# SamsungLabs/fcaf3d

Hardware: AMD Instinct MI355X
Metric: scenes/sec fwd+bwd, ScanNet 100k-pt 2cm voxels, 1/2/4/8 MI355X (higher is better)
Workload: dtype f32

## Files before the change

### fcaf3d_amd/csrc/conv.hip

```cpp
#include "fc_common.h"
#include "../../include/fcaf3d_hip.h"
#ifdef FC_TRACE
__device__ unsigned long long* g_trace_buf_lds;
__device__ int g_trace_cap_lds;
extern "C" int fc_debug_trace_lds(unsigned long long* buf, int cap) {
  FC_HIP(hipMemcpyToSymbol(HIP_SYMBOL(g_trace_buf_lds), &buf, sizeof(buf)));
  FC_HIP(hipMemcpyToSymbol(HIP_SYMBOL(g_trace_cap_lds), &cap, sizeof(cap)));
  return FC_OK;
}
#define TR_BUF g_trace_buf_lds
#define TR_CAP g_trace_cap_lds
#endif
#include "fc_trace.h"

typedef float f32x16 __attribute__((ext_vector_type(16)));
typedef float f32x2 __attribute__((ext_vector_type(2)));
typedef float f32x4 __attribute__((ext_vector_type(4)));

__device__ __attribute__((aligned(16))) float g_zero_row[64];

__device__ int g_fc_prio;
extern "C" int fc_debug_set_prio(int mode) {
  FC_HIP(hipMemcpyToSymbol(HIP_SYMBOL(g_fc_prio), &mode, sizeof(mode)));
  return FC_OK;
// ... 149 lines not shown
  *reinterpret_cast<f32x4*>(out + o * Cout + c4 * 4) = a;
}

__host__ __device__ static inline int fc_stat_rb(int64_t n) { return n <= 1024 ? 16 : (n <= 4096 ? 64 : 32); }

__device__ __forceinline__ void stat_block_reduce(f32x4 a1, f32x4 a2, float* __restrict__ stats, int C, f32x4* sm ) {
  const int lane = threadIdx.x & 15, rl = threadIdx.x >> 4;
  sm[(rl * 2 + 0) * 16 + lane] = a1;
  sm[(rl * 2 + 1) * 16 + lane] = a2;
  __syncthreads();
  if (rl < 2) {
    f32x4 t = {0.f, 0.f, 0.f, 0.f};
#pragma unroll
    for (int q = 0; q < 16; ++q) t += sm[(q * 2 + rl) * 16 + lane];
    *reinterpret_cast<f32x4*>(stats + ((int64_t)blockIdx.x * 2 + rl) * C + blockIdx.y * 64 + lane * 4) = t;
  }
}

struct StatCh { f32x4 mu, is, ga, be; bool bwd, from_y, has_add; int act; };
__device__ __forceinline__ StatCh stat_channels(const X6Epi& epi, int c) {
  StatCh p;
  p.bwd = epi.bn_x != nullptr;
  p.act = epi.act;
  p.from_y = p.bwd && epi.bn_y != nullptr && epi.act != 0;
  p.has_add = p.bwd && epi.add != nullptr;
  p.mu = f32x4{0.f, 0.f, 0.f, 0.f}; p.is = f32x4{1.f, 1.f, 1.f, 1.f}; p.ga = p.is; p.be = p.mu;
  if (p.bwd) {
    p.mu = *reinterpret_cast<const f32x4*>(epi.mean + c);
    const f32x4 va = *reinterpret_cast<const f32x4*>(epi.var + c);
#pragma unroll
    for (int j = 0; j < 4; ++j) p.is[j] = 1.f / sqrtf(va[j] + epi.eps);
    if (epi.gamma) p.ga = *reinterpret_cast<const f32x4*>(epi.gamma + c);
    if (epi.beta) p.be = *reinterpret_cast<const f32x4*>(epi.beta + c);
  }
  return p;
}
__device__ __forceinline__ void stat_accumulate(const StatCh& p, const X6Epi& epi, const f32x4& a, int64_t at, f32x4& a1, f32x4& a2) {
  f32x4 xv = {0.f, 0.f, 0.f, 0.f}, av = xv, yv = xv;
  if (p.bwd) xv = *reinterpret_cast<const f32x4*>(epi.bn_x + at);
  if (p.has_add) av = *reinterpret_cast<const f32x4*>(epi.add + at);
  if (p.from_y) yv = *reinterpret_cast<const f32x4*>(epi.bn_y + at);
#pragma unroll
  for (int j = 0; j < 4; ++j) {
    float t1, t2;
    x6_epi_terms(p.bwd, p.bwd ? av[j] + a[j] : a[j], xv[j], p.mu[j], p.is[j], p.ga[j], p.be[j], p.act, p.from_y, yv[j], t1, t2);
    a1[j] += t1;
    a2[j] += t2;
  }
}

__global__ __launch_bounds__(256) void k_sum_parts_stats(const float* __restrict__ part, float* __restrict__ out, int64_t n, int C, int S,
                                                         int RB, X6Epi epi) {
  __shared__ f32x4 sm[16 * 2 * 16];
  const int lane = threadIdx.x & 15, rl = threadIdx.x >> 4;
  const int64_t r0 = (int64_t)blockIdx.x * RB;
  const int c = blockIdx.y * 64 + lane * 4;
  const StatCh p = stat_channels(epi, c);
  f32x4 a1 = {0.f, 0.f, 0.f, 0.f}, a2 = a1;
  for (int64_t r = r0 + rl; r < r0 + RB && r < n; r += 16) {
    f32x4 a = *reinterpret_cast<const f32x4*>(part + r * C + c);
    for (int z = 1; z < S; ++z) a += *reinterpret_cast<const f32x4*>(part + ((int64_t)z * n + r) * C + c);
    *reinterpret_cast<f32x4*>(out + r * C + c) = a;
    stat_accumulate(p, epi, a, r * C + c, a1, a2);
  }
  stat_block_reduce(a1, a2, epi.stats, C, sm);
}

__global__ __launch_bounds__(256) void k_sum_pairs_stats(const float* __restrict__ part, const int* __restrict__ pos, float* __restrict__ out,
                                                         int64_t n_out, int K, int Cout, int RB, X6Epi epi) {
  __shared__ f32x4 sm[16 * 2 * 16];
  const int lane = threadIdx.x & 15, rl = threadIdx.x >> 4;
  const int64_t r0 = (int64_t)blockIdx.x * RB;
  const int c = blockIdx.y * 64 + lane * 4;
  const StatCh p = stat_channels(epi, c);
  f32x4 a1 = {0.f, 0.f, 0.f, 0.f}, a2 = a1;
  const int64_t rend = (r0 + RB < n_out) ? r0 + RB : n_out;
  for (int64_t o = r0 + rl; o < rend; o += 32) {
    const int64_t o2 = o + 16;
    const bool two = o2 < rend;
    f32x4 a = {0.f, 0.f, 0.f, 0.f}, b = a;
    for (int k0 = 0; k0 < K; k0 += 9) {
      int j[9], j2[9];
#pragma unroll
      for (int u = 0; u < 9; ++u) {
        j[u] = k0 + u < K ? pos[(int64_t)(k0 + u) * n_out + o] : -1;
        j2[u] = (two && k0 + u < K) ? pos[(int64_t)(k0 + u) * n_out + o2] : -1;
      }
      f32x4 v[9], v2[9];
#pragma unroll
      for (int u = 0; u < 9; ++u) {
        const float* src = j[u] >= 0 ? part + ((int64_t)(k0 + u) * n_out + j[u]) * Cout + c : g_zero_row + lane * 4;
        const float* src2 = j2[u] >= 0 ? part + ((int64_t)(k0 + u) * n_out + j2[u]) * Cout + c : g_zero_row + lane * 4;
        v[u] = *reinterpret_cast<const f32x4*>(src);
        v2[u] = *reinterpret_cast<const f32x4*>(src2);
      }
#pragma unroll
      for (int u = 0; u < 9; ++u) {
        if (j[u] >= 0) a += v[u];
        if (j2[u] >= 0) b += v2[u];
      }
    }
    *reinterpret_cast<f32x4*>(out + o * Cout + c) = a;
    stat_accumulate(p, epi, a, o * Cout + c, a1, a2);
    if (two) {
      *reinterpret_cast<f32x4*>(out + o2 * Cout + c) = b;
      stat_accumulate(p, epi, b, o2 * Cout + c, a1, a2);
    }
  }
  stat_block_reduce(a1, a2, epi.stats, Cout, sm);
}

static_assert(STEM_CIN == 3 && STEM_COUT == 64 && BK == 32, "conv_route.h spells these shapes out");

struct ConvArgs {
  const float *in, *W; const int *nbr, *out_index, *cnt; float* dst;
  int64_t n_rows; int K, Cin, Cout; X6Epi epi; hipStream_t stream;
};
#define FC_LAUNCH(...) __VA_ARGS__<<<grid, 256, 0, a.stream>>>(a.in, a.W, a.nbr, a.out_index, a.cnt, a.dst, a.n_rows, a.K, a.Cin, a.Cout)
#define FC_LAUNCH_EPI(...) __VA_ARGS__<<<grid, 256, 0, a.stream>>>(a.in, a.W, a.nbr, a.out_index, a.cnt, a.dst, a.n_rows, a.K, a.Cin, a.Cout, a.epi)

template <int BM, int BN, int WM>
static void launch_conv_fp32(const ConvRoute& r, const ConvArgs& a, dim3 grid) {
#define FC_LAUNCH_MFMA(KERNEL)                                                                                              \
  do { if (r.wsrc == FC_WSRC_FP32_T) FC_LAUNCH(KERNEL<BM, BN, 32, true, WM, true>); else if (a.nbr) FC_LAUNCH(KERNEL<BM, BN, 32, true, WM>); \
       else FC_LAUNCH(KERNEL<BM, BN, 32, false, WM>); } while (0)
  if (r.family == FC_FAM_MFMA) FC_LAUNCH_MFMA(k_conv_mfma);
  if constexpr (BM >= 128) {
    if (r.family == FC_FAM_MFMA_P) FC_LAUNCH_MFMA(k_conv_mfma_p);
    if (r.family == FC_FAM_GLDS) { if (a.nbr) FC_LAUNCH(k_conv_glds<BM, BN, true, WM>); else FC_LAUNCH(k_conv_glds<BM, BN, false, WM>); }
  }
#undef FC_LAUNCH_MFMA
}

template <int BM, int BN, int WM>
static void launch_conv_x6(const ConvRoute& r, const ConvArgs& a, dim3 grid) {
  if (r.family == FC_FAM_H3R) {
    if constexpr (BM == 128) {
      if (r.buf) FC_LAUNCH_EPI(k_conv_h3r<BN, true, true>);
      else if (a.nbr) FC_LAUNCH_EPI(k_conv_h3r<BN, true, false>);
      else FC_LAUNCH_EPI(k_conv_h3r<BN, false, false>);
    }
  } else if (r.wsrc == FC_WSRC_FP32_T) FC_LAUNCH_EPI(k_conv_x6<BM, BN, true, WM, 1>);
  else if (r.wsrc == FC_WSRC_FP32) { if (a.nbr) FC_LAUNCH_EPI(k_conv_x6<BM, BN, true, WM, 0>); else FC_LAUNCH_EPI(k_conv_x6<BM, BN, false, WM, 0>); }
  else if (r.mode == FC_MODE_BF16 || r.buf) {
    if constexpr (BM == 128) {
      if (r.mode == FC_MODE_BF16) { if (a.nbr) FC_LAUNCH_EPI(k_conv_x6<128, BN, true, 2, 2, 1>); else FC_LAUNCH_EPI(k_conv_x6<128, BN, false, 2, 2, 1>); }
      else if (r.mode == FC_MODE_H3) FC_LAUNCH_EPI(k_conv_x6<128, BN, true, 2, 2, 2, true>);
      else FC_LAUNCH_EPI(k_conv_x6<128, BN, true, 2, 2, 0, true>);
    }
  } else if (r.mode == FC_MODE_H3) { if (a.nbr) FC_LAUNCH_EPI(k_conv_x6<BM, BN, true, WM, 2, 2>); else FC_LAUNCH_EPI(k_conv_x6<BM, BN, false, WM, 2, 2>); }
  else { if (a.nbr) FC_LAUNCH_EPI(k_conv_x6<BM, BN, true, WM, 2>); else FC_LAUNCH_EPI(k_conv_x6<BM, BN, false, WM, 2>); }
}

static int launch_conv(const ConvRoute& r, const ConvArgs& a) {
  const dim3 grid(r.grid[0], r.grid[1], r.grid[2]);
  if (r.family == FC_FAM_STEM) {
    const size_t smem = (size_t)(STEM_ROWS * STEM_FWD_LDA + 96 * 64) * sizeof(float);
    k_stem_fwd<<<(unsigned)fc_cdiv(a.n_rows, STEM_ROWS), 256, smem, a.stream>>>(a.in, a.W, a.nbr, a.dst, nullptr, a.n_rows, a.K);
  } else if (r.family == FC_FAM_FMA) {
    k_conv_fma<<<(unsigned)fc_cdiv(a.n_rows * a.Cout, 256), 256, 0, a.stream>>>(a.in, a.W, a.nbr, a.dst, a.n_rows, a.K, a.Cin, a.Cout, r.wsrc == FC_WSRC_FP32_T ? 1 : 0);
  } else {
#define FC_TILE(BM, BN, WM) do { if (r.family >= FC_FAM_X6) launch_conv_x6<BM, BN, WM>(r, a, grid); else launch_conv_fp32<BM, BN, WM>(r, a, grid); } while (0)
    if (r.bm == 256) FC_TILE(256, 64, 4);
    else if (r.bm == 128 && r.bn == 128) FC_TILE(128, 128, 2);
    else if (r.bm == 128) FC_TILE(128, 64, 2);
    else if (r.bn == 128) launch_conv_fp32<64, 128, 2>(r, a, grid);
    else launch_conv_fp32<64, 64, 2>(r, a, grid);
#undef FC_TILE
  }
  FC_CHECK_LAUNCH();
  return FC_OK;
}
#undef FC_LAUNCH
#undef FC_LAUNCH_EPI

extern "C" {

int fc_conv_fwd_route(int64_t n_in, int64_t n_out, int K, int Cin, int Cout, int flags, int table_kind, int64_t live_tiles, int* out) {
  if (!out || n_in < 0 || n_out < 0 || K < 1 || Cin < 1 || Cout < 1) return FC_EINVAL;
  const ConvRoute r = conv_route({n_in, n_out, K, Cin, Cout}, flags, table_kind, live_tiles, route_env());
  const int f[16] = {r.family, r.bm, r.bn, r.wm, r.S, r.wsrc, r.mode, r.buf, r.epi, (int)r.grid[0], (int)r.grid[1], (int)r.grid[2]};
  for (int i = 0; i < 16; ++i) out[i] = f[i];
  return r.family == FC_FAM_INVALID ? FC_EINVAL : FC_OK;
}

int64_t fc_conv_fwd_ws_bytes(int64_t n_out, int K, int Cin, int Cout, int flags) {
  const ConvRoute r = conv_route({n_out, n_out, K, Cin, Cout}, flags, FC_TABLE_DENSE, 0, route_env());
  return r.S > 1 ? (int64_t)r.S * n_out * Cout * (int64_t)sizeof(float) : 0;
}

int64_t fc_conv_fwd_pairs_ws_bytes(int64_t n_out, int K, int Cout) {
  return (int64_t)K * n_out * Cout * (int64_t)sizeof(float);
}

int64_t fc_conv_stats_blocks(int64_t n_out, int K, int Cin, int Cout, int flags, int pairs) {
  if (n_out < 1) return 0;
  const ConvRoute r = conv_route({n_out, n_out, K, Cin, Cout}, flags, pairs ? FC_TABLE_PAIRS : FC_TABLE_DENSE, 0, route_env());
  if (r.epi == FC_EPI_NONE) return 0;
  return r.epi == FC_EPI_SUM ? fc_cdiv(n_out, fc_stat_rb(n_out)) : fc_cdiv(n_out, r.bm);
}

static int conv_impl(const float* in, const float* W, const int* nbr, const int* out_index, const int* cnt, const int* pos, float* out,
                     int64_t n_in, int64_t n_out, int K, int Cin, int Cout, int64_t live_tiles, int flags, void* ws, int64_t ws_bytes,
                     hipStream_t stream, const X6Epi* epi) {
  AmaxHintScope hint_scope;
  if (n_in < 0 || n_out < 0 || K < 1 || Cin < 1 || Cout < 1) return FC_EINVAL;
  if (n_out == 0 && !cnt) return epi ? FC_EINVAL : FC_OK;
  if (out_index && !nbr) return FC_EINVAL;
  const int table = cnt ? FC_TABLE_PAIRS : out_index ? FC_TABLE_SORTED : nbr ? FC_TABLE_DENSE : FC_TABLE_NONE;
  const ConvRoute r = conv_route({n_in, n_out, K, Cin, Cout}, flags, table | (epi ? FC_TABLE_STATS : 0), live_tiles, route_env());
  if (r.family == FC_FAM_INVALID) return FC_EINVAL;
  if (n_out == 0) return FC_OK;
  ConvArgs a = {in, W, nbr, out_index, cnt, out, n_out, K, Cin, Cout, {}, stream};
  if (r.family == FC_FAM_STEM || r.family == FC_FAM_FMA) return launch_conv(r, a);
  const bool parts = cnt || r.S > 1;
  if (parts && ws_bytes < (int64_t)r.S * n_out * Cout * (int64_t)sizeof(float)) return FC_EWS;
  if (parts) a.dst = (float*)ws;
  if (epi && r.epi == FC_EPI_KERNEL) a.epi = *epi;
  int rc = FC_OK;
  if (r.mode == FC_MODE_H3) rc = operand_amax(in, n_in * (int64_t)Cin, 0, stream, &a.epi.amax_in);
  if (rc == FC_OK) rc = launch_conv(r, a);
  if (rc != FC_OK || !parts) return rc;
  const int rb = fc_stat_rb(n_out);
  const dim3 sgrid((unsigned)fc_cdiv(n_out, rb), Cout / 64);
  if (cnt && epi) k_sum_pairs_stats<<<sgrid, 256, 0, stream>>>(a.dst, pos, out, n_out, K, Cout, rb, *epi);
  else if (cnt) k_sum_pairs<<<(unsigned)fc_cdiv(n_out * (Cout / 4), 256), 256, 0, stream>>>(a.dst, pos, out, n_out, K, Cout);
  else if (epi) k_sum_parts_stats<<<sgrid, 256, 0, stream>>>(a.dst, out, n_out, Cout, r.S, rb, *epi);
  else k_sum_parts<<<(unsigned)fc_cdiv(n_out * Cout / 4, 256), 256, 0, stream>>>(a.dst, out, n_out * Cout / 4, r.S);
  FC_CHECK_LAUNCH();
  return FC_OK;
}

static int conv_pairs_impl(const float* in, const float* W, const int* pair_in, const int* pair_cnt, const int* pair_pos, float* out,
                           int64_t n_in, int64_t n_out, int K, int Cin, int Cout, int64_t live_tiles, int flags, void* ws,
                           int64_t ws_bytes, hipStream_t stream, const X6Epi* epi) {
  if (!pair_in || !pair_cnt || !pair_pos || K > 65535) return FC_EINVAL;
  return conv_impl(in, W, pair_in, nullptr, pair_cnt, pair_pos, out, n_in, n_out, K, Cin, Cout, live_tiles, flags, ws, ws_bytes, stream, epi);
}

static X6Epi stats_epi(float* stats, const float* bn_x = nullptr, const float* mean = nullptr, const float* var = nullptr, const float* gamma = nullptr,
                       const float* beta = nullptr, float eps = 0.f, int act = 0, const float* add = nullptr, const float* bn_y = nullptr) {
  return {stats, bn_x, mean, var, gamma, beta, eps, act, add, bn_y, nullptr};
}

int fc_conv_fwd(const float* in, const float* W, const int* nbr, const int* out_index, float* out, int64_t n_in,
                int64_t n_out, int K, int Cin, int Cout, int flags, void* ws, int64_t ws_bytes, hipStream_t stream) {
  return conv_impl(in, W, nbr, out_index, nullptr, nullptr, out, n_in, n_out, K, Cin, Cout, 0, flags, ws, ws_bytes, stream, nullptr);
}

int fc_conv_fwd_stats(const float* in, const float* W, const int* nbr, const int* out_index, float* out, int64_t n_in,
                      int64_t n_out, int K, int Cin, int Cout, int flags, void* ws, int64_t ws_bytes, float* stats,
                      hipStream_t stream) {
  const X6Epi e = stats_epi(stats);
  return conv_impl(in, W, nbr, out_index, nullptr, nullptr, out, n_in, n_out, K, Cin, Cout, 0, flags, ws, ws_bytes, stream, stats ? &e : nullptr);
}

int fc_conv_fwd_bn_bwd_stats(const float* in, const float* W, const int* nbr, const int* out_index, float* out, int64_t n_in,
                             int64_t n_out, int K, int Cin, int Cout, int flags, void* ws, int64_t ws_bytes, float* stats,
                             const float* bn_x, const float* mean, const float* var, const float* gamma, const float* beta, float eps,
                             int act, const float* add, const float* bn_y, hipStream_t stream) {
  if (!stats || !bn_x || !mean || !var || act < 0 || act > 2) return FC_EINVAL;
  const X6Epi e = stats_epi(stats, bn_x, mean, var, gamma, beta, eps, act, add, bn_y);
  return conv_impl(in, W, nbr, out_index, nullptr, nullptr, out, n_in, n_out, K, Cin, Cout, 0, flags, ws, ws_bytes, stream, &e);
}

int fc_conv_fwd_pairs_tiles(const float* in, const float* W, const int* pair_in, const int* pair_cnt, const int* pair_pos,
                            float* out, int64_t n_in, int64_t n_out, int K, int Cin, int Cout, int64_t live_tiles, int flags,
                            void* ws, int64_t ws_bytes, hipStream_t stream) {
  return conv_pairs_impl(in, W, pair_in, pair_cnt, pair_pos, out, n_in, n_out, K, Cin, Cout, live_tiles, flags, ws, ws_bytes, stream, nullptr);
}

int fc_conv_fwd_pairs_tiles_stats(const float* in, const float* W, const int* pair_in, const int* pair_cnt, const int* pair_pos,
                                  float* out, int64_t n_in, int64_t n_out, int K, int Cin, int Cout, int64_t live_tiles, int flags,
                                  void* ws, int64_t ws_bytes, float* stats, hipStream_t stream) {
  const X6Epi e = stats_epi(stats);
  return conv_pairs_impl(in, W, pair_in, pair_cnt, pair_pos, out, n_in, n_out, K, Cin, Cout, live_tiles, flags, ws, ws_bytes, stream,
                         stats ? &e : nullptr);
}

int fc_conv_fwd_pairs_tiles_bn_bwd_stats(const float* in, const float* W, const int* pair_in, const int* pair_cnt, const int* pair_pos,
                                         float* out, int64_t n_in, int64_t n_out, int K, int Cin, int Cout, int64_t live_tiles, int flags,
                                         void* ws, int64_t ws_bytes, float* stats, const float* bn_x, const float* mean,
                                         const float* var, const float* gamma, const float* beta, float eps, int act,
                                         const float* add, const float* bn_y, hipStream_t stream) {
  if (!stats || !bn_x || !mean || !var || act < 0 || act > 2) return FC_EINVAL;
  const X6Epi e = stats_epi(stats, bn_x, mean, var, gamma, beta, eps, act, add, bn_y);
  return conv_pairs_impl(in, W, pair_in, pair_cnt, pair_pos, out, n_in, n_out, K, Cin, Cout, live_tiles, flags, ws, ws_bytes, stream, &e);
}

int fc_conv_fwd_pairs(const float* in, const float* W, const int* pair_in, const int* pair_cnt, const int* pair_pos,
                      float* out, int64_t n_in, int64_t n_out, int K, int Cin, int Cout, int flags, void* ws,
                      int64_t ws_bytes, hipStream_t stream) {
  return fc_conv_fwd_pairs_tiles(in, W, pair_in, pair_cnt, pair_pos, out, n_in, n_out, K, Cin, Cout, 0, flags, ws, ws_bytes, stream);
}

int64_t fc_x6_weight_image_bytes(int K, int R, int C) { return (int64_t)K * R * C * 6; }

int fc_x6_weight_image(const float* W, void* img, int K, int R, int C, int transposed, hipStream_t stream) {
  if (K < 1 || R < 32 || C < 64 || R % 32 != 0 || C % 64 != 0) return FC_EINVAL;
  const int64_t total = (int64_t)K * (R / 32) * (C / 64) * 256;
  const unsigned nb = (unsigned)fc_cdiv(total, 256);
  if (split_mode() == 2) {
    FC_HIP(hipMemsetAsync((char*)img + 4 * X6_IMG_AMAX_WORD, 0, FC_AMAX_SLOT_BYTES, stream));
    k_x6_weight_image<3><<<nb, 256, 0, stream>>>(W, (u32x4*)img, K, R, C, transposed);
    k_x6_weight_image<2><<<nb, 256, 0, stream>>>(W, (u32x4*)img, K, R, C, transposed);
  } else {
    k_x6_weight_image<0><<<nb, 256, 0, stream>>>(W, (u32x4*)img, K, R, C, transposed);
  }
  FC_CHECK_LAUNCH();
  return FC_OK;
}

int64_t fc_x6_amax_units(void) { return X6_AMAX_UNITS; }

int fc_x6_weight_images_passes(const int64_t* desc, int n, int64_t total_blocks, const int64_t* amax_chunks, int64_t amax_blocks,
                               int passes, hipStream_t stream) {
  if (!desc || n < 1 || total_blocks < 1 || total_blocks > 0x7fffffffll || amax_blocks < 0 || amax_blocks > 0x7fffffffll ||
      (amax_blocks && !amax_chunks))
    return FC_EINVAL;
  const long long* d = reinterpret_cast<const long long*>(desc);
  if (split_mode() == 2) {
    if (passes & 1) k_x6_weight_images<4><<<(unsigned)fc_cdiv(n, 4), 256, 0, stream>>>(d, n);
    if ((passes & 2) && amax_blocks)
      k_x6_weight_amax<X6_AMAX_UNITS><<<(unsigned)amax_blocks, 256, 0, stream>>>(d, reinterpret_cast<const long long*>(amax_chunks));
    if (passes & 4) k_x6_weight_images<2><<<(unsigned)total_blocks, 256, 0, stream>>>(d, n);
  } else if (passes & 4) {
    k_x6_weight_images<0><<<(unsigned)total_blocks, 256, 0, stream>>>(d, n);
  }
  FC_CHECK_LAUNCH();
  return FC_OK;
}

int fc_x6_weight_images(const int64_t* desc, int n, int64_t total_blocks, const int64_t* amax_chunks, int64_t amax_blocks,
                        hipStream_t stream) {
  return fc_x6_weight_images_passes(desc, n, total_blocks, amax_chunks, amax_blocks, 7, stream);
}

}

__global__ void k_wgrad_reduce(const float* __restrict__ part, float* __restrict__ gW, int64_t elems, int S) {
  int64_t i = (int64_t)blockIdx.x * blockDim.x + threadIdx.x;
  if (i >= elems) return;
  float acc = 0.f;
  for (int s = 0; s < S; ++s) acc += part[(int64_t)s * elems + i];
  gW[i] = acc;
}

template <int G>
__global__ __launch_bounds__(256) void k_wgrad_reduce4(const float* __restrict__ part, float* __restrict__ gW, int64_t elems4, int S) {
  __shared__ f32x4 red[256];
  constexpr int COLS = 256 / G;
  const int col = threadIdx.x % COLS, g = threadIdx.x / COLS;
  const int64_t i = (int64_t)blockIdx.x * COLS + col;
  const int per = (S + G - 1) / G;
  const int s0 = g * per, s1 = (s0 + per < S) ? s0 + per : S;
  f32x4 a = {0.f, 0.f, 0.f, 0.f};
  if (i < elems4) {
    const f32x4* src = reinterpret_cast<const f32x4*>(part) + i;
    int sl = s0;
    for (; sl + 4 <= s1; sl += 4) {
      const f32x4 v0 = src[(int64_t)sl * elems4], v1 = src[(int64_t)(sl + 1) * elems4];
      const f32x4 v2 = src[(int64_t)(sl + 2) * elems4], v3 = src[(int64_t)(sl + 3) * elems4];
      a += v0; a += v1; a += v2; a += v3;
    }
    for (; sl < s1; ++sl) a += src[(int64_t)sl * elems4];
  }
  if (G == 1) {
    if (i < elems4) reinterpret_cast<f32x4*>(gW)[i] = a;
    return;
  }
  red[threadIdx.x] = a;
  __syncthreads();
  if (g == 0 && i < elems4) {
    for (int q = 1; q < G; ++q) a += red[q * COLS + col];
    reinterpret_cast<f32x4*>(gW)[i] = a;
  }
}

__global__ void k_transpose_w(const float* __restrict__ W, float* __restrict__ Wt, int K, int Cin, int Cout) {
  __shared__ float tile[32][33];
  int k = blockIdx.z;
  int ci0 = blockIdx.y * 32, co0 = blockIdx.x * 32;
  int tx = threadIdx.x & 31, ty = threadIdx.x >> 5;
  for (int j = ty; j < 32; j += 8) {
    int ci = ci0 + j, co = co0 + tx;
    tile[j][tx] = (ci < Cin && co < Cout) ? W[((int64_t)k * Cin + ci) * Cout + co] : 0.f;
  }
  __syncthreads();
  for (int j = ty; j < 32; j += 8) {
    int co = co0 + j, ci = ci0 + tx;
    if (ci < Cin && co < Cout) Wt[((int64_t)k * Cout + co) * Cin + ci] = tile[tx][j];
  }
}

struct WgradArgs {
  const float *in, *gout; const int *nbr, *row_index, *cnt; float* part;
  int64_t n_out; int K, Cin, Cout; const unsigned *amax_in, *amax_gout; hipStream_t stream;
};
#define FC_LAUNCH(...) __VA_ARGS__<<<grid, 256, 0, a.stream>>>(a.in, a.gout, a.nbr, a.row_index, a.cnt, a.part, a.n_out, a.K, a.Cin, a.Cout, r.rps)
#define FC_LAUNCH_X6T(...) __VA_ARGS__<<<grid, 256, 0, a.stream>>>(a.in, a.gout, a.nbr, a.row_index, a.cnt, a.part, a.n_out, a.K, a.Cin, a.Cout, r.rps, a.amax_in, a.amax_gout, r.wbuf)
#define FC_LAUNCH_TABLE(...) __VA_ARGS__<<<grid, 256, 0, a.stream>>>(a.in, a.gout, a.nbr, a.part, a.n_out, a.K, a.Cin, a.Cout, r.rps)

template <int BM, int BN, int KO, bool PAIRS>
static void launch_wgrad_x6t(const WgradRoute& r, const WgradArgs& a, dim3 grid) {
  if (r.mode == FC_MODE_BF16) FC_LAUNCH_X6T(k_wgrad_x6t<BM, BN, KO, PAIRS, 1>);
  else if (r.mode == FC_MODE_H3) FC_LAUNCH_X6T(k_wgrad_x6t<BM, BN, KO, PAIRS, 2>);
  else FC_LAUNCH_X6T(k_wgrad_x6t<BM, BN, KO, PAIRS>);
}

template <int BM, int BN>
static void launch_wgrad_tile(const WgradRoute& r, const WgradArgs& a, dim3 grid) {
  const bool pairs = r.table == FC_TABLE_PAIRS;
  if (r.family == FC_WFAM_X6T) { if (pairs) launch_wgrad_x6t<BM, BN, 1, true>(r, a, grid); else launch_wgrad_x6t<BM, BN, 1, false>(r, a, grid); }
  else if (r.family == FC_WFAM_MFMA && !pairs && r.bkr == 32) { if (a.nbr) FC_LAUNCH(k_wgrad_mfma<BM, BN, true, 32, false>); else FC_LAUNCH(k_wgrad_mfma<BM, BN, false, 32, false>); }
  else if constexpr (BM == 64) {
    if (r.family == FC_WFAM_MFMA) { if (pairs) FC_LAUNCH(k_wgrad_mfma<64, BN, true, 32, true>); else FC_LAUNCH(k_wgrad_mfma<64, BN, true, 64, false>); }
    else if (pairs) FC_LAUNCH(k_wgrad_mfma_p<BN, true, true>);
    else if (a.nbr) FC_LAUNCH(k_wgrad_mfma_p<BN, true, false>);
    else FC_LAUNCH(k_wgrad_mfma_p<BN, false, false>);
  }
}

static int launch_wgrad(const WgradRoute& r, const WgradArgs& a) {
  const dim3 grid((unsigned)r.S, r.grid_y);
  const bool wide = r.bn == 128;
  if (r.family == FC_WFAM_STEM) {
    const size_t smem = (size_t)(STEM_ROWS * STEM_JP + STEM_ROWS * 64) * sizeof(float);
    k_stem_wgrad<<<(unsigned)r.S, 256, smem, a.stream>>>(a.in, a.gout, a.nbr, a.part, a.n_out, a.K, r.rps);
  } else if (r.family == FC_WFAM_FMA) FC_LAUNCH_TABLE(k_wgrad_fma);
  else if (r.family == FC_WFAM_MULTI) { if (wide) FC_LAUNCH_TABLE(k_wgrad_multi<128, WGRAD_KO>); else FC_LAUNCH_TABLE(k_wgrad_multi<64, WGRAD_KO>); }
  else if (r.ko == WGRAD_KO) { if (wide) launch_wgrad_x6t<64, 128, WGRAD_KO, false>(r, a, grid); else launch_wgrad_x6t<64, 64, WGRAD_KO, false>(r, a, grid); }
  else if (r.bm == 128) { if (wide) launch_wgrad_tile<128, 128>(r, a, grid); else launch_wgrad_tile<128, 64>(r, a, grid); }
  else { if (wide) launch_wgrad_tile<64, 128>(r, a, grid); else launch_wgrad_tile<64, 64>(r, a, grid); }
  FC_CHECK_LAUNCH();
  return FC_OK;
}
#undef FC_LAUNCH
#undef FC_LAUNCH_X6T
#undef FC_LAUNCH_TABLE

extern "C" {

static int wgrad_reduce(const float* part, float* gW, int64_t elems, int S, hipStream_t stream) {
  if (elems % 4 == 0) {
    const int64_t e4 = elems / 4;
    if (S >= 64) k_wgrad_reduce4<16><<<(unsigned)fc_cdiv(e4, 16), 256, 0, stream>>>(part, gW, e4, S);
    else if (S >= 16) k_wgrad_reduce4<4><<<(unsigned)fc_cdiv(e4, 64), 256, 0, stream>>>(part, gW, e4, S);
    else k_wgrad_reduce4<1><<<(unsigned)fc_cdiv(e4, 256), 256, 0, stream>>>(part, gW, e4, S);
  } else {
    k_wgrad_reduce<<<(unsigned)fc_cdiv(elems, 256), 256, 0, stream>>>(part, gW, elems, S);
  }
  FC_CHECK_LAUNCH();
  return FC_OK;
}

int fc_stem_conv_fwd(const float* in, const float* W, const int* nbr, float* out, float* col, int64_t n_in, int64_t n_out,
                     int K, hipStream_t stream) {
  if (n_in < 0 || n_out < 0 || K < 1 || K > 27 || !nbr) return FC_EINVAL;
  if (n_out == 0) return FC_OK;
  size_t smem = (size_t)(STEM_ROWS * STEM_FWD_LDA + 96 * 64) * sizeof(float);
  k_stem_fwd<<<(unsigned)fc_cdiv(n_out, STEM_ROWS), 256, smem, stream>>>(in, W, nbr, out, col, n_out, K);
  FC_CHECK_LAUNCH();
  return FC_OK;
}

static void stem_col_plan(int64_t n_out, int* S, int64_t* rps) {
  int64_t r = fc_cdiv(fc_cdiv(n_out > 0 ? n_out : 1, 192), STEM_ROWS) * STEM_ROWS;
  *rps = r;
  *S = (int)fc_cdiv(n_out > 0 ? n_out : 1, r);
}

int64_t fc_stem_conv_wgrad_ws_bytes(int64_t n_out, int K) {
  int S; int64_t rps;
  stem_col_plan(n_out, &S, &rps);
  return (int64_t)S * K * STEM_CIN * STEM_COUT * (int64_t)sizeof(float);
}

int fc_stem_conv_wgrad(const float* col, const float* gout, float* gW, int64_t n_out, int K, void* ws, int64_t ws_bytes,
                       hipStream_t stream) {
  if (n_out < 0 || K < 1 || K > 27) return FC_EINVAL;
  const int64_t elems = (int64_t)K * STEM_CIN * STEM_COUT;
  if (n_out == 0) {
    FC_HIP(hipMemsetAsync(gW, 0, elems * sizeof(float), stream));
    return FC_OK;
  }
  int S; int64_t rps;
  stem_col_plan(n_out, &S, &rps);
  if (ws_bytes < (int64_t)S * elems * (int64_t)sizeof(float)) return FC_EWS;
  float* part = (S == 1) ? gW : (float*)ws;
  size_t smem = (size_t)(STEM_ROWS * STEM_JP + STEM_ROWS * 64) * sizeof(float);
  k_stem_wgrad_col<<<(unsigned)S, 256, smem, stream>>>(col, gout, part, n_out, K, rps);
  FC_CHECK_LAUNCH();
  if (S > 1) return wgrad_reduce(part, gW, elems, S, stream);
  return FC_OK;
}

int fc_conv_wgrad_route(int64_t n_in, int64_t n_out, int K, int Cin, int Cout, int flags, int table_kind, int* out) {
  if (!out || n_in < 0 || n_out < 0 || K < 1 || Cin < 1 || Cout < 1) return FC_EINVAL;
  const WgradRoute r = wgrad_route({n_in, n_out, K, Cin, Cout}, flags, table_kind, route_env());
  const int f[16] = {r.family, r.bm, r.bn, r.ko, r.bkr, r.table, r.mode, r.S, (int)(r.rps < 0x7fffffff ? r.rps : 0x7fffffff), r.wbuf, (int)r.grid_y};
  for (int i = 0; i < 16; ++i) out[i] = f[i];
  return r.family == FC_WFAM_INVALID ? FC_EINVAL : FC_OK;
}

int64_t fc_conv_wgrad_ws_bytes(int64_t n_out, int K, int Cin, int Cout, int flags) {
  int S = 0;
  for (int table : {FC_TABLE_NONE, FC_TABLE_DENSE, FC_TABLE_PAIRS}) {
    const WgradRoute r = wgrad_route({n_out, n_out, K, Cin, Cout}, flags, table, route_env());
    if (r.family != FC_WFAM_INVALID && r.S > S) S = r.S;
  }
  return (int64_t)S * K * Cin * Cout * (int64_t)sizeof(float);
}

static int conv_wgrad_impl(const float* in, const float* gout, const int* nbr, const int* row_index, const int* cnt,
                           float* gW, int64_t n_in, int64_t n_out, int K, int Cin, int Cout, int flags, void* ws,
                           int64_t ws_bytes, hipStream_t stream) {
  AmaxHintScope hint_scope;
  if (n_in < 0 || n_out < 0 || K < 1 || Cin < 1 || Cout < 1) return FC_EINVAL;
  const int64_t elems = (int64_t)K * Cin * Cout;
  if (n_out == 0) { FC_HIP(hipMemsetAsync(gW, 0, elems * sizeof(float), stream)); return FC_OK; }
  const WgradRoute r = wgrad_route({n_in, n_out, K, Cin, Cout}, flags, cnt ? FC_TABLE_PAIRS : nbr ? FC_TABLE_DENSE : FC_TABLE_NONE, route_env());
  if (r.family == FC_WFAM_INVALID) return FC_EINVAL;
  if (ws_bytes < (int64_t)r.S * elems * (int64_t)sizeof(float)) return FC_EWS;
  WgradArgs a = {in, gout, nbr, row_index, cnt, (r.S == 1) ? gW : (float*)ws, n_out, K, Cin, Cout, nullptr, nullptr, stream};
  int rc = FC_OK;
  if (r.mode == FC_MODE_H3) {
    rc = operand_amax(in, n_in * (int64_t)Cin, 0, stream, &a.amax_in);
    if (rc == FC_OK) rc = operand_amax(gout, n_out * (int64_t)Cout, 1, stream, &a.amax_gout);
  }
  if (rc == FC_OK) rc = launch_wgrad(r, a);
  if (rc == FC_OK && r.S > 1) rc = wgrad_reduce(a.part, gW, elems, r.S, stream);
  return rc;
}

int fc_conv_wgrad(const float* in, const float* gout, const int* nbr, const int* row_index, float* gW, int64_t n_in,
                  int64_t n_out, int K, int Cin, int Cout, int flags, void* ws, int64_t ws_bytes, hipStream_t stream) {
  if (row_index) return FC_EINVAL;
  return conv_wgrad_impl(in, gout, nbr, nullptr, nullptr, gW, n_in, n_out, K, Cin, Cout, flags, ws, ws_bytes, stream);
}

int fc_conv_wgrad_pairs(const float* in, const float* gout, const int* pair_in, const int* pair_out, const int* pair_cnt,
                        float* gW, int64_t n_in, int64_t n_out, int K, int Cin, int Cout, int flags, void* ws,
                        int64_t ws_bytes, hipStream_t stream) {
  if (!pair_in || !pair_out || !pair_cnt) return FC_EINVAL;
  return conv_wgrad_impl(in, gout, pair_in, pair_out, pair_cnt, gW, n_in, n_out, K, Cin, Cout, flags, ws, ws_bytes, stream);
}

int fc_transpose_weight(const float* W, float* Wt, int K, int Cin, int Cout, hipStream_t stream) {
  if (K < 1 || Cin < 1 || Cout < 1 || K > 65535) return FC_EINVAL;
  dim3 grid((unsigned)fc_cdiv(Cout, 32), (unsigned)fc_cdiv(Cin, 32), (unsigned)K);
  k_transpose_w<<<grid, 256, 0, stream>>>(W, Wt, K, Cin, Cout);
  FC_CHECK_LAUNCH();
  return FC_OK;
}

}
```

### fcaf3d_amd/csrc/conv_stem.h

```cpp
#pragma once

#define STEM_CIN 3
#define STEM_COUT 64
#define STEM_ROWS 64
#define STEM_FWD_LDA 97
#define STEM_COL_LD 84
__global__ __launch_bounds__(256) void k_stem_fwd(const float* __restrict__ in, const float* __restrict__ W,
                                                  const int* __restrict__ nbr, float* __restrict__ out,
                                                  float* __restrict__ col, int64_t n_out, int K) {
  extern __shared__ float sm[];
  constexpr int SLD = STEM_FWD_LDA;
  const int KC = K * STEM_CIN;
  float* in_s = sm;
  float* W_s = sm + STEM_ROWS * SLD;
  const int tid = threadIdx.x, lane = tid & 63, wave = tid >> 6;
  const int r = lane & 31, h = lane >> 5, wr = wave >> 1, wc = wave & 1;
  const int64_t m0 = (int64_t)blockIdx.x * STEM_ROWS;
  for (int t = tid; t < STEM_ROWS * (SLD - KC); t += 256) {
    int row = t / (SLD - KC), c = KC + t % (SLD - KC);
    in_s[row * SLD + c] = 0.f;
  }
  for (int t = tid; t < STEM_ROWS * K; t += 256) {
    int k = t / STEM_ROWS, row = t % STEM_ROWS;
    int64_t o = m0 + row;
    int64_t oc = o < n_out ? o : n_out - 1;
    int i = nbr[(int64_t)k * n_out + oc];
    if (o >= n_out) i = -1;
    const float* src = i < 0 ? g_zero_row : in + (int64_t)i * 3;
    float a = src[0], b = src[1], c = src[2];
    in_s[row * SLD + k * 3] = a; in_s[row * SLD + k * 3 + 1] = b; in_s[row * SLD + k * 3 + 2] = c;
  }
  for (int t = tid; t < 96 * 16; t += 256) {
    f32x4 v = {0.f, 0.f, 0.f, 0.f};
    if (t < KC * 16) v = reinterpret_cast<const f32x4*>(W)[t];
    reinterpret_cast<f32x4*>(W_s)[t] = v;
  }
  __syncthreads();
  if (col) {
    for (int t = tid; t < STEM_ROWS * (STEM_COL_LD / 4); t += 256) {
      const int row = t / (STEM_COL_LD / 4), c = (t % (STEM_COL_LD / 4)) * 4;
      const int64_t o = m0 + row;
      if (o < n_out) {
        const float* sp = in_s + row * SLD + c;
        f32x4 v = {sp[0], sp[1], sp[2], sp[3]};
        *reinterpret_cast<f32x4*>(col + o * STEM_COL_LD + c) = v;
      }
    }
  }
  f32x16 acc;
#pragma unroll
  for (int e = 0; e < 16; ++e) acc[e] = 0.f;
  const float* ap = in_s + (wr * 32 + r) * SLD + h;
  const float* bp = W_s + h * 64 + wc * 32 + r;
#pragma unroll 8
  for (int sidx = 0; sidx < 48; ++sidx)
    acc = __builtin_amdgcn_mfma_f32_32x32x2f32(ap[2 * sidx], bp[2 * sidx * 64], acc, 0, 0, 0);
#pragma unroll
  for (int e = 0; e < 16; ++e) {
    int64_t o = m0 + wr * 32 + (e & 3) + 8 * (e >> 2) + 4 * h;
    if (o < n_out) out[o * 64 + wc * 32 + r] = acc[e];
  }
}

#define STEM_JP 96
__global__ __launch_bounds__(256) void k_stem_wgrad(const float* __restrict__ in, const float* __restrict__ gout,
                                                    const int* __restrict__ nbr, float* __restrict__ part, int64_t n_out,
                                                    int K, int64_t rows_per_block) {
  extern __shared__ float sm[];
  const int KC = K * STEM_CIN;
  float* in_s = sm;
  float* g_s = sm + STEM_ROWS * STEM_JP;
  const int tid = threadIdx.x, lane = tid & 63, wave = tid >> 6;
  const int r = lane & 31, h = lane >> 5;
  const int64_t r_begin = (int64_t)blockIdx.x * rows_per_block;
  int64_t r_end = r_begin + rows_per_block;
  if (r_end > n_out) r_end = n_out;
  for (int t = tid; t < STEM_ROWS * STEM_JP; t += 256) in_s[t] = 0.f;
  f32x16 acc[3][2];
#pragma unroll
  for (int i = 0; i < 3; ++i)
#pragma unroll
    for (int j = 0; j < 2; ++j)
#pragma unroll
      for (int e = 0; e < 16; ++e) acc[i][j][e] = 0.f;
  constexpr int NG = (STEM_ROWS * 27 + 255) / 256;
  float pa[NG][3];
  f32x4 pg[4];
  auto load_chunk = [&](int64_t rb) {
    int idx[NG];
#pragma unroll
    for (int u = 0; u < NG; ++u) {
      const int t = tid + 256 * u;
      const int k = t / STEM_ROWS, row = t % STEM_ROWS;
      const int64_t o = rb + row;
      const int64_t oc = o < r_end ? o : r_end - 1;
      const int kk = k < K ? k : K - 1;
      int i = nbr[(int64_t)kk * n_out + oc];
      idx[u] = (o < r_end && k < K) ? i : -1;
    }
#pragma unroll
    for (int u = 0; u < 4; ++u) {
      const int t = tid + 256 * u;
      const int64_t o = rb + (t >> 4);
      const float* gp = o < r_end ? gout + o * 64 + (t & 15) * 4 : g_zero_row;
      pg[u] = *reinterpret_cast<const f32x4*>(gp);
    }
#pragma unroll
    for (int u = 0; u < NG; ++u) {
      const float* src = idx[u] < 0 ? g_zero_row : in + (int64_t)idx[u] * 3;
      pa[u][0] = src[0]; pa[u][1] = src[1]; pa[u][2] = src[2];
    }
  };
  if (r_begin < r_end) load_chunk(r_begin);
  for (int64_t rb = r_begin; rb < r_end; rb += STEM_ROWS) {
    __syncthreads();
#pragma unroll
    for (int u = 0; u < NG; ++u) {
      const int t = tid + 256 * u;
      const int k = t / STEM_ROWS, row = t % STEM_ROWS;
      if (k < K) {
        in_s[row * STEM_JP + k * 3] = pa[u][0]; in_s[row * STEM_JP + k * 3 + 1] = pa[u][1]; in_s[row * STEM_JP + k * 3 + 2] = pa[u][2];
      }
    }
#pragma unroll
    for (int u = 0; u < 4; ++u) reinterpret_cast<f32x4*>(g_s)[tid + 256 * u] = pg[u];
    __syncthreads();
    load_chunk(rb + STEM_ROWS < r_end ? rb + STEM_ROWS : rb);
#pragma unroll
    for (int sidx = 0; sidx < 8; ++sidx) {
      const int row = wave * 16 + 2 * sidx + h;
      float a[3], b[2];
#pragma unroll
      for (int i = 0; i < 3; ++i) a[i] = in_s[row * STEM_JP + i * 32 + r];
#pragma unroll
      for (int j = 0; j < 2; ++j) b[j] = g_s[row * 64 + j * 32 + r];
#pragma unroll
      for (int i = 0; i < 3; ++i)
#pragma unroll
        for (int j = 0; j < 2; ++j) acc[i][j] = __builtin_amdgcn_mfma_f32_32x32x2f32(a[i], b[j], acc[i][j], 0, 0, 0);
    }
  }
  __syncthreads();
  float* red = sm;
  for (int w = 0; w < 4; ++w) {
    if (wave == w) {
#pragma unroll
      for (int i = 0; i < 3; ++i)
#pragma unroll
        for (int j = 0; j < 2; ++j)
#pragma unroll
          for (int e = 0; e < 16; ++e) {
            int jj = i * 32 + (e & 3) + 8 * (e >> 2) + 4 * h, co = j * 32 + r;
            float v = acc[i][j][e];
            if (w > 0) v += red[jj * 64 + co];
            red[jj * 64 + co] = v;
          }
    }
    __syncthreads();
  }
  float* dst = part + (int64_t)blockIdx.x * KC * 64;
  for (int t = tid; t < KC * 64; t += 256) dst[t] = red[t];
}

__global__ __launch_bounds__(256) void k_stem_wgrad_col(const float* __restrict__ col, const float* __restrict__ gout,
                                                        float* __restrict__ part, int64_t n_out, int K, int64_t rows_per_block) {
  extern __shared__ float sm[];
  const int KC = K * STEM_CIN;
  float* in_s = sm;
  float* g_s = sm + STEM_ROWS * STEM_JP;
  const int tid = threadIdx.x, lane = tid & 63, wave = tid >> 6;
  const int r = lane & 31, h = lane >> 5;
  const int64_t r_begin = (int64_t)blockIdx.x * rows_per_block;
  int64_t r_end = r_begin + rows_per_block;
  if (r_end > n_out) r_end = n_out;
  for (int t = tid; t < STEM_ROWS * STEM_JP; t += 256) in_s[t] = 0.f;
  f32x16 acc[3][2];
#pragma unroll
  for (int i = 0; i < 3; ++i)
#pragma unroll
    for (int j = 0; j < 2; ++j)
#pragma unroll
      for (int e = 0; e < 16; ++e) acc[i][j][e] = 0.f;
  constexpr int NC = (STEM_ROWS * (STEM_COL_LD / 4) + 255) / 256;
  f32x4 pc[NC], pg[4];
  auto load_chunk = [&](int64_t rb) {
#pragma unroll
    for (int u = 0; u < NC; ++u) {
      const int t = tid + 256 * u;
      const int row = t / (STEM_COL_LD / 4), c = (t % (STEM_COL_LD / 4)) * 4;
      const int64_t o = rb + row;
      const float* cp = (o < r_end && row < STEM_ROWS) ? col + o * STEM_COL_LD + c : g_zero_row;
      pc[u] = *reinterpret_cast<const f32x4*>(cp);
    }
#pragma unroll
    for (int u = 0; u < 4; ++u) {
      const int t = tid + 256 * u;
      const int64_t o = rb + (t >> 4);
      const float* gp = o < r_end ? gout + o * 64 + (t & 15) * 4 : g_zero_row;
      pg[u] = *reinterpret_cast<const f32x4*>(gp);
    }
  };
  if (r_begin < r_end) load_chunk(r_begin);
  for (int64_t rb = r_begin; rb < r_end; rb += STEM_ROWS) {
    __syncthreads();
#pragma unroll
    for (int u = 0; u < NC; ++u) {
      const int t = tid + 256 * u;
      const int row = t / (STEM_COL_LD / 4), c = (t % (STEM_COL_LD / 4)) * 4;
      if (row < STEM_ROWS) *reinterpret_cast<f32x4*>(&in_s[row * STEM_JP + c]) = pc[u];
    }
#pragma unroll
    for (int u = 0; u < 4; ++u) reinterpret_cast<f32x4*>(g_s)[tid + 256 * u] = pg[u];
    __syncthreads();
    load_chunk(rb + STEM_ROWS < r_end ? rb + STEM_ROWS : rb);
#pragma unroll
    for (int sidx = 0; sidx < 8; ++sidx) {
      const int row = wave * 16 + 2 * sidx + h;
      float a[3], b[2];
#pragma unroll
      for (int i = 0; i < 3; ++i) a[i] = in_s[row * STEM_JP + i * 32 + r];
#pragma unroll
      for (int j = 0; j < 2; ++j) b[j] = g_s[row * 64 + j * 32 + r];
#pragma unroll
      for (int i = 0; i < 3; ++i)
#pragma unroll
        for (int j = 0; j < 2; ++j) acc[i][j] = __builtin_amdgcn_mfma_f32_32x32x2f32(a[i], b[j], acc[i][j], 0, 0, 0);
    }
  }
  __syncthreads();
  float* red = sm;
  for (int w = 0; w < 4; ++w) {
    if (wave == w) {
#pragma unroll
      for (int i = 0; i < 3; ++i)
#pragma unroll
        for (int j = 0; j < 2; ++j)
#pragma unroll
          for (int e = 0; e < 16; ++e) {
            int jj = i * 32 + (e & 3) + 8 * (e >> 2) + 4 * h, co = j * 32 + r;
            float v = acc[i][j][e];
            if (w > 0) v += red[jj * 64 + co];
            red[jj * 64 + co] = v;
          }
    }
    __syncthreads();
  }
  float* dst = part + (int64_t)blockIdx.x * KC * 64;
  for (int t = tid; t < KC * 64; t += 256) dst[t] = red[t];
}
```

Measured before the change: 540.4.

## Make stem forward persistent with prefetched gathers and register-pipeline stem wgrad

The stem forward kernel becomes persistent, launching a grid capped at a fixed number of workgroups per CU. Each workgroup loops over tiles, prefetching neighbor indices and gathered inputs for upcoming tiles into registers and deferring the output store so it overlaps the next tile's work. The stem weight-gradient kernel drops its LDS staging and loads col/gout straight into registers with a three-deep software pipeline feeding the MFMAs, and uses less shared memory. The cost is higher register pressure, which may lower occupancy, plus more per-thread scattered scalar global loads.

```diff
diff --git a/fcaf3d_amd/csrc/conv.hip b/fcaf3d_amd/csrc/conv.hip
--- a/fcaf3d_amd/csrc/conv.hip
+++ b/fcaf3d_amd/csrc/conv.hip
@@ -325,11 +325,39 @@
   else { if (a.nbr) FC_LAUNCH_EPI(k_conv_x6<BM, BN, true, WM, 2>); else FC_LAUNCH_EPI(k_conv_x6<BM, BN, false, WM, 2>); }
 }
 
+static int stem_fwd_resident(int* wgs) {
+  static int g_cus[16] = {};
+  static std::mutex mu;
+  int dev = 0;
+  FC_HIP(hipGetDevice(&dev));
+  if (dev < 0 || dev >= 16) return FC_EINVAL;
+  std::lock_guard<std::mutex> lock(mu);
+  if (!g_cus[dev]) {
+    int cus = 0;
+    FC_HIP(hipDeviceGetAttribute(&cus, hipDeviceAttributeMultiprocessorCount, dev));
+    if (cus < 1) return FC_EINVAL;
+    g_cus[dev] = cus;
+  }
+  *wgs = g_cus[dev] * STEM_FWD_WGS_PER_CU;
+  return FC_OK;
+}
+
+static int launch_stem_fwd(const float* in, const float* W, const int* nbr, float* out, float* col, int64_t n_out, int K,
+                           hipStream_t stream) {
+  int wgs = 0;
+  const int rc = stem_fwd_resident(&wgs);
+  if (rc != FC_OK) return rc;
+  const int64_t tiles = fc_cdiv(n_out, STEM_ROWS);
+  const size_t smem = (size_t)(STEM_ROWS * STEM_FWD_LDA + 96 * 64) * sizeof(float);
+  k_stem_fwd<<<(unsigned)(tiles < wgs ? tiles : wgs), 256, smem, stream>>>(in, W, nbr, out, col, n_out, K);
+  return FC_OK;
+}
+
 static int launch_conv(const ConvRoute& r, const ConvArgs& a) {
   const dim3 grid(r.grid[0], r.grid[1], r.grid[2]);
   if (r.family == FC_FAM_STEM) {
-    const size_t smem = (size_t)(STEM_ROWS * STEM_FWD_LDA + 96 * 64) * sizeof(float);
-    k_stem_fwd<<<(unsigned)fc_cdiv(a.n_rows, STEM_ROWS), 256, smem, a.stream>>>(a.in, a.W, a.nbr, a.dst, nullptr, a.n_rows, a.K);
+    const int rc = launch_stem_fwd(a.in, a.W, a.nbr, a.dst, nullptr, a.n_rows, a.K, a.stream);
+    if (rc != FC_OK) return rc;
   } else if (r.family == FC_FAM_FMA) {
     k_conv_fma<<<(unsigned)fc_cdiv(a.n_rows * a.Cout, 256), 256, 0, a.stream>>>(a.in, a.W, a.nbr, a.dst, a.n_rows, a.K, a.Cin, a.Cout, r.wsrc == FC_WSRC_FP32_T ? 1 : 0);
   } else {
@@ -631,10 +659,15 @@
                      int K, hipStream_t stream) {
   if (n_in < 0 || n_out < 0 || K < 1 || K > 27 || !nbr) return FC_EINVAL;
   if (n_out == 0) return FC_OK;
-  size_t smem = (size_t)(STEM_ROWS * STEM_FWD_LDA + 96 * 64) * sizeof(float);
-  k_stem_fwd<<<(unsigned)fc_cdiv(n_out, STEM_ROWS), 256, smem, stream>>>(in, W, nbr, out, col, n_out, K);
-  FC_CHECK_LAUNCH();
-  return FC_OK;
+  const int rc = launch_stem_fwd(in, W, nbr, out, col, n_out, K, stream);
+  if (rc != FC_OK) return rc;
+  FC_CHECK_LAUNCH();
+  return FC_OK;
+}
+
+int fc_debug_stem_fwd_grid(void) {
+  int wgs = 0;
+  return stem_fwd_resident(&wgs) == FC_OK ? wgs : -1;
 }
 
 static void stem_col_plan(int64_t n_out, int* S, int64_t* rps) {
@@ -661,8 +694,7 @@
   stem_col_plan(n_out, &S, &rps);
   if (ws_bytes < (int64_t)S * elems * (int64_t)sizeof(float)) return FC_EWS;
   float* part = (S == 1) ? gW : (float*)ws;
-  size_t smem = (size_t)(STEM_ROWS * STEM_JP + STEM_ROWS * 64) * sizeof(float);
-  k_stem_wgrad_col<<<(unsigned)S, 256, smem, stream>>>(col, gout, part, n_out, K, rps);
+  k_stem_wgrad_col<<<(unsigned)S, 256, STEM_WCOL_SMEM, stream>>>(col, gout, part, n_out, K, rps);
   FC_CHECK_LAUNCH();
   if (S > 1) return wgrad_reduce(part, gW, elems, S, stream);
   return FC_OK;
diff --git a/fcaf3d_amd/csrc/conv_stem.h b/fcaf3d_amd/csrc/conv_stem.h
--- a/fcaf3d_amd/csrc/conv_stem.h
+++ b/fcaf3d_amd/csrc/conv_stem.h
@@ -5,6 +5,7 @@
 #define STEM_ROWS 64
 #define STEM_FWD_LDA 97
 #define STEM_COL_LD 84
+#define STEM_FWD_WGS_PER_CU 3
 __global__ __launch_bounds__(256) void k_stem_fwd(const float* __restrict__ in, const float* __restrict__ W,
                                                   const int* __restrict__ nbr, float* __restrict__ out,
                                                   float* __restrict__ col, int64_t n_out, int K) {
@@ -15,51 +16,84 @@
   float* W_s = sm + STEM_ROWS * SLD;
   const int tid = threadIdx.x, lane = tid & 63, wave = tid >> 6;
   const int r = lane & 31, h = lane >> 5, wr = wave >> 1, wc = wave & 1;
-  const int64_t m0 = (int64_t)blockIdx.x * STEM_ROWS;
+  const int64_t n_tiles = (n_out + STEM_ROWS - 1) / STEM_ROWS, step = gridDim.x;
   for (int t = tid; t < STEM_ROWS * (SLD - KC); t += 256) {
     int row = t / (SLD - KC), c = KC + t % (SLD - KC);
     in_s[row * SLD + c] = 0.f;
-  }
-  for (int t = tid; t < STEM_ROWS * K; t += 256) {
-    int k = t / STEM_ROWS, row = t % STEM_ROWS;
-    int64_t o = m0 + row;
-    int64_t oc = o < n_out ? o : n_out - 1;
-    int i = nbr[(int64_t)k * n_out + oc];
-    if (o >= n_out) i = -1;
-    const float* src = i < 0 ? g_zero_row : in + (int64_t)i * 3;
-    float a = src[0], b = src[1], c = src[2];
-    in_s[row * SLD + k * 3] = a; in_s[row * SLD + k * 3 + 1] = b; in_s[row * SLD + k * 3 + 2] = c;
   }
   for (int t = tid; t < 96 * 16; t += 256) {
     f32x4 v = {0.f, 0.f, 0.f, 0.f};
     if (t < KC * 16) v = reinterpret_cast<const f32x4*>(W)[t];
     reinterpret_cast<f32x4*>(W_s)[t] = v;
   }
-  __syncthreads();
-  if (col) {
-    for (int t = tid; t < STEM_ROWS * (STEM_COL_LD / 4); t += 256) {
-      const int row = t / (STEM_COL_LD / 4), c = (t % (STEM_COL_LD / 4)) * 4;
-      const int64_t o = m0 + row;
-      if (o < n_out) {
-        const float* sp = in_s + row * SLD + c;
-        f32x4 v = {sp[0], sp[1], sp[2], sp[3]};
-        *reinterpret_cast<f32x4*>(col + o * STEM_COL_LD + c) = v;
-      }
-    }
-  }
+  constexpr int NG = (STEM_ROWS * 27 + 255) / 256;
+  int idx[NG];
+  float pa[NG][3];
+  auto load_idx = [&](int64_t tile) {
+    const int64_t o = tile * STEM_ROWS + lane;
+    const int64_t oc = o < n_out ? o : n_out - 1;
+#pragma unroll
+    for (int u = 0; u < NG; ++u) {
+      const int k = wave + 4 * u;
+      const int kk = k < K ? k : K - 1;
+      const int i = nbr[(int64_t)kk * n_out + oc];
+      idx[u] = i | ((o < n_out && k < K) ? 0 : -1);
+    }
+  };
+  auto gather = [&]() {
+#pragma unroll
+    for (int u = 0; u < NG; ++u) {
+      const float* src = idx[u] < 0 ? g_zero_row : in + (int64_t)idx[u] * 3;
+      pa[u][0] = src[0]; pa[u][1] = src[1]; pa[u][2] = src[2];
+    }
+  };
   f32x16 acc;
-#pragma unroll
-  for (int e = 0; e < 16; ++e) acc[e] = 0.f;
-  const float* ap = in_s + (wr * 32 + r) * SLD + h;
-  const float* bp = W_s + h * 64 + wc * 32 + r;
+  auto store_out = [&](int64_t m0) {
+#pragma unroll
+    for (int e = 0; e < 16; ++e) {
+      int64_t o = m0 + wr * 32 + (e & 3) + 8 * (e >> 2) + 4 * h;
+      if (o < n_out) out[o * 64 + wc * 32 + r] = acc[e];
+    }
+  };
+  const int64_t last = n_tiles - 1;
+  int64_t tile = blockIdx.x;
+  int64_t prev_m0 = -1;
+  load_idx(tile);
+  gather();
+  load_idx(tile + step < n_tiles ? tile + step : last);
+  for (; tile < n_tiles; tile += step) {
+    const int64_t m0 = tile * STEM_ROWS;
+    __syncthreads();
+#pragma unroll
+    for (int u = 0; u < NG; ++u) {
+      const int k = wave + 4 * u;
+      in_s[lane * SLD + k * 3] = pa[u][0]; in_s[lane * SLD + k * 3 + 1] = pa[u][1]; in_s[lane * SLD + k * 3 + 2] = pa[u][2];
+    }
+    __syncthreads();
+    if (prev_m0 >= 0) store_out(prev_m0);
+    if (col) {
+      for (int t = tid; t < STEM_ROWS * (STEM_COL_LD / 4); t += 256) {
+        const int row = t / (STEM_COL_LD / 4), c = (t % (STEM_COL_LD / 4)) * 4;
+        const int64_t o = m0 + row;
+        if (o < n_out) {
+          const float* sp = in_s + row * SLD + c;
+          f32x4 v = {sp[0], sp[1], sp[2], sp[3]};
+          *reinterpret_cast<f32x4*>(col + o * STEM_COL_LD + c) = v;
+        }
+      }
+    }
+    gather();
+    load_idx(tile + 2 * step < n_tiles ? tile + 2 * step : last);
+#pragma unroll
+    for (int e = 0; e < 16; ++e) acc[e] = 0.f;
+    const float* ap = in_s + (wr * 32 + r) * SLD + h;
+    const float* bp = W_s + h * 64 + wc * 32 + r;
 #pragma unroll 8
-  for (int sidx = 0; sidx < 48; ++sidx)
-    acc = __builtin_amdgcn_mfma_f32_32x32x2f32(ap[2 * sidx], bp[2 * sidx * 64], acc, 0, 0, 0);
-#pragma unroll
-  for (int e = 0; e < 16; ++e) {
-    int64_t o = m0 + wr * 32 + (e & 3) + 8 * (e >> 2) + 4 * h;
-    if (o < n_out) out[o * 64 + wc * 32 + r] = acc[e];
-  }
+    for (int sidx = 0; sidx < 48; ++sidx)
+      acc = __builtin_amdgcn_mfma_f32_32x32x2f32(ap[2 * sidx], bp[2 * sidx * 64], acc, 0, 0, 0);
+    prev_m0 = m0;
+  }
+  if (prev_m0 >= 0) store_out(prev_m0);
 }
 
 #define STEM_JP 96
@@ -162,18 +196,16 @@
   for (int t = tid; t < KC * 64; t += 256) dst[t] = red[t];
 }
 
+#define STEM_WCOL_SMEM (STEM_JP * 64 * sizeof(float))
 __global__ __launch_bounds__(256) void k_stem_wgrad_col(const float* __restrict__ col, const float* __restrict__ gout,
                                                         float* __restrict__ part, int64_t n_out, int K, int64_t rows_per_block) {
   extern __shared__ float sm[];
   const int KC = K * STEM_CIN;
-  float* in_s = sm;
-  float* g_s = sm + STEM_ROWS * STEM_JP;
   const int tid = threadIdx.x, lane = tid & 63, wave = tid >> 6;
   const int r = lane & 31, h = lane >> 5;
   const int64_t r_begin = (int64_t)blockIdx.x * rows_per_block;
   int64_t r_end = r_begin + rows_per_block;
   if (r_end > n_out) r_end = n_out;
-  for (int t = tid; t < STEM_ROWS * STEM_JP; t += 256) in_s[t] = 0.f;
   f32x16 acc[3][2];
 #pragma unroll
   for (int i = 0; i < 3; ++i)
@@ -181,53 +213,48 @@
     for (int j = 0; j < 2; ++j)
 #pragma unroll
       for (int e = 0; e < 16; ++e) acc[i][j][e] = 0.f;
-  constexpr int NC = (STEM_ROWS * (STEM_COL_LD / 4) + 255) / 256;
-  f32x4 pc[NC], pg[4];
-  auto load_chunk = [&](int64_t rb) {
-#pragma unroll
-    for (int u = 0; u < NC; ++u) {
-      const int t = tid + 256 * u;
-      const int row = t / (STEM_COL_LD / 4), c = (t % (STEM_COL_LD / 4)) * 4;
-      const int64_t o = rb + row;
-      const float* cp = (o < r_end && row < STEM_ROWS) ? col + o * STEM_COL_LD + c : g_zero_row;
-      pc[u] = *reinterpret_cast<const f32x4*>(cp);
-    }
-#pragma unroll
-    for (int u = 0; u < 4; ++u) {
-      const int t = tid + 256 * u;
-      const int64_t o = rb + (t >> 4);
-      const float* gp = o < r_end ? gout + o * 64 + (t & 15) * 4 : g_zero_row;
-      pg[u] = *reinterpret_cast<const f32x4*>(gp);
-    }
-  };
-  if (r_begin < r_end) load_chunk(r_begin);
-  for (int64_t rb = r_begin; rb < r_end; rb += STEM_ROWS) {
-    __syncthreads();
-#pragma unroll
-    for (int u = 0; u < NC; ++u) {
-      const int t = tid + 256 * u;
-      const int row = t / (STEM_COL_LD / 4), c = (t % (STEM_COL_LD / 4)) * 4;
-      if (row < STEM_ROWS) *reinterpret_cast<f32x4*>(&in_s[row * STEM_JP + c]) = pc[u];
-    }
-#pragma unroll
-    for (int u = 0; u < 4; ++u) reinterpret_cast<f32x4*>(g_s)[tid + 256 * u] = pg[u];
-    __syncthreads();
-    load_chunk(rb + STEM_ROWS < r_end ? rb + STEM_ROWS : rb);
+  float pa[3][8][3], pb[3][8][2];
+  auto load_chunk = [&](int s, int64_t rb) {
 #pragma unroll
     for (int sidx = 0; sidx < 8; ++sidx) {
-      const int row = wave * 16 + 2 * sidx + h;
-      float a[3], b[2];
-#pragma unroll
-      for (int i = 0; i < 3; ++i) a[i] = in_s[row * STEM_JP + i * 32 + r];
-#pragma unroll
-      for (int j = 0; j < 2; ++j) b[j] = g_s[row * 64 + j * 32 + r];
-#pragma unroll
-      for (int i = 0; i < 3; ++i)
-#pragma unroll
-        for (int j = 0; j < 2; ++j) acc[i][j] = __builtin_amdgcn_mfma_f32_32x32x2f32(a[i], b[j], acc[i][j], 0, 0, 0);
-    }
-  }
-  __syncthreads();
+      const int64_t o = rb + wave * 16 + 2 * sidx + h;
+      const bool ok = o < r_end;
+#pragma unroll
+      for (int i = 0; i < 3; ++i) {
+        const int c = i * 32 + r;
+        const float* cp = (ok && c < STEM_COL_LD) ? col + o * STEM_COL_LD + c : g_zero_row;
+        pa[s][sidx][i] = *cp;
+      }
+#pragma unroll
+      for (int j = 0; j < 2; ++j) {
+        const float* gp = ok ? gout + o * 64 + j * 32 + r : g_zero_row;
+        pb[s][sidx][j] = *gp;
+      }
+    }
+  };
+  auto multiply = [&](int s) {
+#pragma unroll
+    for (int sidx = 0; sidx < 8; ++sidx)
+#pragma unroll
+      for (int i = 0; i < 3; ++i)
+#pragma unroll
+        for (int j = 0; j < 2; ++j) acc[i][j] = __builtin_amdgcn_mfma_f32_32x32x2f32(pa[s][sidx][i], pb[s][sidx][j], acc[i][j], 0, 0, 0);
+  };
+  const int64_t n_chunks = (r_end - r_begin + STEM_ROWS - 1) / STEM_ROWS;
+  int64_t rb = r_begin;
+  load_chunk(0, rb);
+  load_chunk(1, rb + STEM_ROWS);
+  load_chunk(2, rb + 2 * STEM_ROWS);
+  for (int64_t i = 0; i < n_chunks / 3; ++i, rb += 3 * STEM_ROWS) {
+    multiply(0);
+    load_chunk(0, rb + 3 * STEM_ROWS);
+    multiply(1);
+    load_chunk(1, rb + 4 * STEM_ROWS);
+    multiply(2);
+    load_chunk(2, rb + 5 * STEM_ROWS);
+  }
+  if (n_chunks % 3 >= 1) multiply(0);
+  if (n_chunks % 3 == 2) multiply(1);
   float* red = sm;
   for (int w = 0; w < 4; ++w) {
     if (wave == w) {
```

After: 543.3 (median of 6 runs). About the same (+0.5%).
